# JanSpindler/NRC-HPM-Renderer

Hardware: AMD Instinct MI355X
Metric: Msamples/s + ms/frame at 1080p, 256^3 cloud (NRC path) (higher is better)
Workload: dtype f16 (fp16 MFMA operands, fp32 accumulate; fp32 integrator)

## Files before the change

### nrc-hpm-renderer_amd/csrc/nrc_api.hip

```cpp
#include <algorithm>
#include <array>
#include <atomic>
#include <chrono>
#include <cmath>
#include <cstdio>
#include <cstdlib>
#include <cstring>
#include <fstream>
#include <map>
#include <memory>
#include <mutex>
#include <random>
#include <string>
#include <thread>
#include <unordered_map>
#include <vector>

#include <dlfcn.h>
#include <rccl/rccl.h>

#include "nrc_integrator.hpp"
#include "nrc_mlp.hpp"
#include "nrc_checkpoint.hpp"
#include "nrc_occupancy.hpp"
#include "nrc_schedule.hpp"
#include "nrc_volume_keys.hpp"
#include "build_id.h"

namespace nrc {

static thread_local std::string g_last_error;

namespace {
constexpr size_t kGuardBytes = 4096;
struct AllocInfo {
    void* base;
    size_t bytes;
    std::string what;
};
struct AllocRegistry {
    std::mutex mu;
    std::unordered_map<void*, AllocInfo> live;
    bool poison = debug_value("poison_alloc", 0) != 0;
    bool guard = debug_value("guard_alloc", 0) != 0;
    unsigned long long violations = 0;
    std::string first_violation;
};
std::atomic<int> g_live_allocations{0};
AllocRegistry& alloc_registry()
{
    static AllocRegistry r;
    return r;
}
size_t guard_damage(const AllocInfo& a, std::string* where)
{
    std::vector<unsigned char> g(2 * kGuardBytes);
    if (hipMemcpy(g.data(), a.base, kGuardBytes, hipMemcpyDeviceToHost) != hipSuccess) return 0;
    if (hipMemcpy(g.data() + kGuardBytes, (char*)a.base + kGuardBytes + a.bytes, kGuardBytes, hipMemcpyDeviceToHost) != hipSuccess) return 0;
    size_t bad = 0;
    long first = -1;
    for (size_t i = 0; i < g.size(); i++)
        if (g[i] != 0xA5) { bad++; if (first < 0) first = (long)i; }
    if (bad && where)
        *where = a.what + " (" + std::to_string(a.bytes) + " B): " + std::to_string(bad) + " canary bytes overwritten, first at offset " +
                 (first < (long)kGuardBytes ? std::to_string(first - (long)kGuardBytes) : "+" + std::to_string(a.bytes + (size_t)first - kGuardBytes)) ;
    return bad;
}
}

void dev_alloc(void** p, size_t bytes, const char* what)
{
    AllocRegistry& r = alloc_registry();
    if (!r.guard) {
        NRC_HIP(hipMalloc(p, bytes));
        g_live_allocations++;
        if (r.poison && bytes) NRC_HIP(hipMemset(*p, 0xFF, bytes));
        return;
    }
    const size_t padded = (bytes + 255) & ~(size_t)255;
    void* base = nullptr;
    NRC_HIP(hipMalloc(&base, padded + 2 * kGuardBytes));
    NRC_HIP(hipMemset(base, 0xA5, padded + 2 * kGuardBytes));
    *p = (char*)base + kGuardBytes;
    g_live_allocations++;
    if (bytes) NRC_HIP(hipMemset(*p, r.poison ? 0xFF : 0x00, bytes));
    std::lock_guard<std::mutex> lock(r.mu);
    r.live[*p] = AllocInfo{base, bytes, what ? what : ""};
}

void dev_free(void* p)
{
    if (!p) return;
    g_live_allocations--;
    AllocRegistry& r = alloc_registry();
    if (!r.guard) {
        (void)hipFree(p);
        return;
    }
    AllocInfo a{nullptr, 0, ""};
    {
        std::lock_guard<std::mutex> lock(r.mu);
        auto it = r.live.find(p);
        if (it == r.live.end()) { (void)hipFree(p); return; }
        a = it->second;
        r.live.erase(it);
    }
    (void)hipDeviceSynchronize();
    AllocInfo chk = a;
// ... 1099 lines not shown
    unsigned long long* for_launch() const { return on ? d_count.get() : nullptr; }
    void set(bool enable, hipStream_t s) { on = enable; NRC_HIP(hipMemsetAsync(d_count, 0, 8, s)); }
    unsigned long long read(hipStream_t s) const
    {
        unsigned long long v = 0;
        NRC_HIP(hipMemcpyAsync(&v, d_count, 8, hipMemcpyDeviceToHost, s));
        NRC_HIP(hipStreamSynchronize(s));
        return v;
    }
};

struct PinnedRandom {
    float r[4] = {0, 0, 0, 0};
    bool have = false;
    void set(const float* r4) { std::memcpy(r, r4, 16); have = true; }
    bool take(float* frame_random) { if (have) std::memcpy(frame_random, r, 16); return std::exchange(have, false); }
};

static bool path_keys(const SceneDev& scene, uint32_t n_cameras, const nrc_camera* cameras, const float* times, uint32_t frames_per_camera,
                      std::vector<KeyTime>* keys)
{
    if (n_cameras == 0) return false;
    if (cameras == nullptr) fail("render_path: cameras is NULL");
    if (frames_per_camera == 0) fail("render_path: frames_per_camera must be at least 1");
    for (uint32_t i = 0; times != nullptr && i < n_cameras; i++) keys->push_back(scene.key_time(times[i], "render_path_timed"));
    return true;
}

static void export_framebuffer(const char* path, const float* d_rgba, uint32_t w, uint32_t h, hipStream_t s)
{
    std::vector<float> host((size_t)w * h * 4);
    NRC_HIP(hipMemcpyAsync(host.data(), d_rgba, host.size() * 4, hipMemcpyDeviceToHost, s));
    NRC_HIP(hipStreamSynchronize(s));
    write_exr(path, host, w, h);
}

class Renderer {
public:
    Renderer(uint32_t w, uint32_t h, bool blend, const nrc_camera& cam, const nrc_config& cfg, const nrc_scene& scene,
             Cache& cache, const nrc_tile* tile, hipStream_t s)
        : w_(w), h_(h), cam_(to_dev(cam)), cfg_(cfg), cache_(cache), stream_(s), blend_(blend), rng_(cfg.seed)
    {
        if (w == 0 || h == 0) fail("render size must be non-zero");
        if (((size_t)w * h) % 16 != 0) fail("NRC requires inferCount to be a multiple of 16");
        frame_ = make_frame(w, h, tile);
        tile_ = tile ? *tile : nrc_tile{0, 1, w, h, 1};
        prepare_hot_tiles(frame_, &hot_finder_);
        nq_ = query_count(w, h);
        scene_.upload(scene);
        calc_train_subset(cfg.train_batch_count * cache.train_batch_size());
        tg_.spp = cfg.train_spp;
        tg_.ray_length = (cfg.compat_fix & NRC_FIX_Q2_TRAIN_RAY_LEN) ? cfg.train_ray_length : 1u;
        tg_.ring_size = (uint32_t)(cfg.train_ring_buf_size * (float)(tg_.tw * tg_.th));
        const size_t px = (size_t)w * h, T = (size_t)tg_.tw * tg_.th;
        for (GenSet& g : gen_) {
            g.primary = alloc<float>(px * 4, "primary image"); g.info = alloc<float>(px, "info image");
            g.origin = alloc<float>(px * 4, "vertex origin image"); g.dir = alloc<float>(px * 4, "vertex direction image");
            g.infer_in = alloc<float>((size_t)nq_ * 5, "inference queries"); g.infer_out = alloc<float>((size_t)nq_ * 3, "inference radiance");
            if (!debug_switch("no_live_list")) g.live = alloc<uint32_t>((size_t)nq_ + 1, "live-query list");
            g.prep_done.create(); g.comp_done.create();
        }
        d_out_ = alloc<float>(px * 4, "framebuffer");
        if (cfg.self_train > 1u) fail("self_train must be 0 or 1");
        self_train_ = cfg.self_train != 0u;
        const size_t TS = T * tg_.spp;
        for (TrainSet& t : train_) {
            t.train_in = alloc<float>(T * 5, "training inputs"); t.train_target = alloc<float>(T * 3, "training targets");
            if (self_train_) {
                t.tail_q = alloc<float>(TS * 5, "tail queries"); t.tail_rec = alloc<float>(TS * 4, "tail records");
                t.tail_y = alloc<float>(TS * 3, "tail radiance");
            }
            t.infer_done.create(); t.train_done.create();
        }
        if (self_train_) cache.mlp().reserve_side_slot((uint32_t)TS);
        ring_entries_ = std::max<size_t>(T, tg_.ring_size);
        d_ring_ = alloc<uint32_t>(2 + ring_entries_ * 6, "train ring");
        d_scratch_ = alloc<uint32_t>(2 * T + 4, "train-ray scratch");
        fetch_.d_count = alloc<unsigned long long>(1, "fetch counter");
        mask_.d_tile_mask = alloc<uint32_t>(tile_mask_words(w, h), "tile mask");
        static_assert(kFlightStates % 32 == 0, "one bit per state, in whole words");
        mask_.d_flight_bits = alloc<uint32_t>((size_t)kFlightStates / 32 + 2, "flight bits");
        mask_.d_flight_sel = alloc<uint32_t>(1 + kFlightListMax, "flight selection");
        zero_dead_queries_ = debug_switch("zero_dead_queries");
        n_slots_ = camera_slots(w, h);
        if (n_slots_ > kOrderSlotMask) fail("render size: more 8x8 tiles than the launch order can address");
        d_tile_cost_ = alloc<uint32_t>(n_slots_, "tile costs");
        for (auto& o : d_tile_order_) o = alloc<uint32_t>(n_slots_, "tile order");
        {
            std::vector<uint32_t> ident(n_slots_);
            for (uint32_t i = 0; i < n_slots_; i++) ident[i] = i;
            for (auto& o : d_tile_order_) NRC_HIP(hipMemcpy(o, ident.data(), ident.size() * 4, hipMemcpyHostToDevice));
        }
        ev_order_done_ = make_event(hipEventDisableTiming);
        {
            hipDeviceProp_t prop{};
            int dev = 0;
            NRC_HIP(hipGetDevice(&dev));
            NRC_HIP(hipGetDeviceProperties(&prop, dev));
            std::string arch = prop.gcnArchName;
            arch = arch.substr(0, arch.find(':'));
            sched_ = ScheduleTuner(device_xcds() == 8, nrc::schedule_key(arch, prop.multiProcessorCount, device_xcds(), cfg,
                                                                    (unsigned long long)scene.nx * scene.ny * scene.nz, w, h, tile_.global_w,
                                                                    tile_.global_h, cache.train_batch_size(), tg_.ray_length));
        }
        mask_.cam = cam;
        if (!debug_switch("single_stream")) {
            int lo = 0, hi = 0;
            NRC_HIP(hipDeviceGetStreamPriorityRange(&lo, &hi));
            stream_b_ = make_stream(hi);
            stream_c_ = make_stream(hi);
            stream_d_ = make_stream(hi);
            if (train_paths_are_long(tg_)) {
                for (TraceSet& q : trace_) {
                    q.stream = make_stream(hi);
                    q.ev_trace_done = make_event(hipEventDisableTiming);
                    q.ev_staged = make_event(hipEventDisableTiming);
                    q.train_start = alloc<float>(T * 6, "staged start vertices");
                    q.in_stage = alloc<float>(T * 5, "staged training inputs");
                    q.target_stage = alloc<float>(T * 3, "staged training targets");
                    if (self_train_) {
                        q.tail_q_stage = alloc<float>(TS * 5, "staged tail queries");
                        q.tail_rec_stage = alloc<float>(TS * 4, "staged tail records");
                    }
                }
            }
        }
        std::vector<uint32_t> ring(2 + ring_entries_ * 6, 0);
        for (size_t r = 0; r < ring_entries_; r++) { float one = 1.0f; std::memcpy(&ring[2 + 6 * r + 5], &one, 4); }
        NRC_HIP(hipMemcpy(d_ring_, ring.data(), ring.size() * 4, hipMemcpyHostToDevice));
        cache_.init(nq_, gen_[0].infer_in, gen_[0].infer_out, train_[0].train_in, train_[0].train_target, s);
    }

    ~Renderer()
    {
        (void)hipDeviceSynchronize();
        cache_.forget(this);
    }

    void render(bool train, bool may_defer = false, bool mask_tiles = false)
    {
        if (train) cache_.poll_comm();
        if (ev_idx_.must_grow(ev_pool_.size())) {
            std::array<Event, 10> set;
            for (auto& e : set) e = make_event(hipEventDefault);
            ev_pool_.push_back(std::move(set));
        }
        sched_.step(TunerStep{frame_index_, ev_idx_.used, ev_pool_.size(), ev_idx_.last, ev_idx_.epoch, stage_events_, stream_c_ != nullptr}, *this);
        frame_.camera_priority_low = sched_.now().pri != 0 ? 1u : 0u;
        const Event* ev_ = ev_pool_[ev_idx_.take()].data();
        const float blend_factor = 1.0f / (float)blend_index_;
        const bool pinned = pinned_random_.take(frame_.random);
        if (!pinned && have_next_random_) { std::memcpy(frame_.random, next_random_, 16); have_next_random_ = false; }
        else if (!pinned) draw_random(frame_.random);
        if (blend_) blend_index_++;
        hipStream_t A = stream_, B = stream_b_ ? stream_b_ : stream_, Cs = stream_c_ ? stream_c_ : stream_;
        hipStream_t D = stream_d_ ? stream_d_ : B;
        mask_.update(scene_, &frame_, A, mask_tiles);
        const int pp = (int)(frame_index_ & 1u);
        const int gp = (int)(frame_index_ % (uint64_t)kGenSets);
        GenSet& g = gen_[gp];
        TrainSet& t = train_[pp];
        last_gen_ = gp; last_train_ = pp;
        if (frame_index_ >= (uint64_t)kGenSets) {
            if (Cs != A) NRC_HIP(hipStreamWaitEvent(A, g.comp_done.ev, 0));
            if (D != A && Cs == A) NRC_HIP(hipStreamWaitEvent(A, g.prep_done.ev, 0));
        }
        const int tq = (int)(frame_index_ % (uint64_t)kTraceSets);
        TraceSet& q = trace_[tq];
        const bool long_trace = q.stream != nullptr;
        if (long_trace) { if (frame_index_ >= (uint64_t)kTraceSets) NRC_HIP(hipStreamWaitEvent(D, q.ev_staged, 0)); }
        else if (frame_index_ >= 2 && D != B) NRC_HIP(hipStreamWaitEvent(D, t.train_done.ev, 0));
        if (cost_order_ && order_pending_ && frame_index_ >= order_pending_frame_ + (uint64_t)sched_.now().lag) {
            if (D != A) NRC_HIP(hipStreamWaitEvent(A, ev_order_done_, 0));
            order_cur_ ^= 1;
            order_pending_ = false;
        }
        const bool sample_cost = cost_order_ && !order_pending_ && (frame_index_ % kOrderEvery == 0 || order_resample_);
        if (sample_cost) order_resample_ = false;
        frame_.tile_order = cost_order_ ? d_tile_order_[order_cur_].get() : nullptr;
        frame_.tile_cost = sample_cost ? d_tile_cost_.get() : nullptr;
        frame_.tile_cost_keep = order_fresh_ > 0 ? 0u : kOrderKeep;
        if (sample_cost && order_fresh_ > 0) order_fresh_--;
        frame_.hot_front = frame_.hot_n = 0u;
        const bool promote = hot_promote_ && frame_.tile_mask != nullptr && frame_.flight_mode == 1u && frame_.flight_n > 0;
        if (promote) {
            last_hot_predicted_ = next_known_ && std::memcmp(known_random_, frame_.random, 16) == 0;
            last_hot_list_ = promote_hot_tiles(&frame_, &hot_finder_);
            const float* nr = next_random_;
            if (have_hint_) nr = hint_random_;
            else if (!have_next_random_) { draw_random(next_random_); have_next_random_ = true; }
            std::memcpy(known_random_, nr, 16);
        }
        have_hint_ = false;
        next_known_ = promote;
        last_hot_ = promote;
        frame_.live_list = frame_.live_count = nullptr;
        if (g.live != nullptr && cache_.wants_live_list()) {
            frame_.live_count = g.live;
            frame_.live_list = frame_.live_count + 1;
        }
        frame_.skip_dead_queries = (!zero_dead_queries_ && frame_.live_list != nullptr && (cache_.encodes_in_kernel() || cache_.model_has_grid())) ? 1u : 0u;
        {
            LaunchTailScope tail(A, ev_[1], ev_[0]);
            launch_gen_rays(scene_.d, cam_, frame_, cfg_.primary_ray_length, cfg_.primary_ray_prob, g.primary, g.info, g.origin, g.dir,
                            g.infer_in, fetch_.for_launch(), tg_, full_vertex_images_, A);
            tail.finish();
        }
        if (D != A) NRC_HIP(hipStreamWaitEvent(D, ev_[1], 0));
        if (Cs != A) NRC_HIP(hipStreamWaitEvent(Cs, ev_[1], 0));
        const hipEvent_t prep_done = g.prep_done.select(stage_events_, ev_[2]);
        const bool pre_encode = train && D != B && frame_index_ >= 2 && !long_trace && cache_.can_pre_encode(this);
        const bool self_train = train && self_train_ && tg_.ring_size > 0;
        float* tail_q = self_train ? (long_trace ? q.tail_q_stage : t.tail_q).get() : nullptr;
        float* tail_rec = self_train ? (long_trace ? q.tail_rec_stage : t.tail_rec).get() : nullptr;
        {
            LaunchTailScope tail(D);
            if (!pre_encode) tail.arm(prep_done);
            launch_prep_train(scene_.d, frame_, tg_, g.info, g.origin, g.dir, d_ring_, d_scratch_, long_trace ? q.in_stage : t.train_in,
                              t.train_target, D, long_trace ? q.train_start.get() : nullptr, long_trace ? nullptr : tail_q,
                              long_trace ? nullptr : tail_rec);
            if (pre_encode) {
                cache_.pre_encode(t.train_in, pp, D);
                tail.arm(prep_done);
            }
            tail.finish();
        }
        if (long_trace) {
            hipStream_t T = q.stream;
            NRC_HIP(hipStreamWaitEvent(T, prep_done, 0));
            {
                LaunchTailScope tail(T, q.ev_trace_done);
                launch_train_trace(scene_.d, frame_, tg_, q.train_start, q.target_stage, T, tail_q, tail_rec);
                tail.finish();
            }
            NRC_HIP(hipStreamWaitEvent(B, q.ev_trace_done, 0));
            const size_t nT = (size_t)tg_.tw * tg_.th;
            NRC_HIP(hipMemcpyAsync(t.train_in, q.in_stage, nT * 5 * sizeof(float), hipMemcpyDeviceToDevice, B));
            if (!self_train) {
                NRC_HIP(hipMemcpyAsync(t.train_target, q.target_stage, nT * 3 * sizeof(float), hipMemcpyDeviceToDevice, B));
                NRC_HIP(hipEventRecord(q.ev_staged, B));
            }
        } else if (B != D) NRC_HIP(hipStreamWaitEvent(B, prep_done, 0));
        if (sample_cost) {
            LaunchTailScope tail(D, ev_order_done_);
            launch_tile_order(d_tile_cost_, n_slots_, d_tile_order_[order_cur_ ^ 1], w_, D,
                              sched_.xcd_ok() ? (uint32_t)sched_.now().window : 0u, hot_promote_ ? kHotTilesMax / 4u : 0u);
            tail.finish();
            order_pending_ = true;
            order_pending_frame_ = frame_index_;
        }
        if (pending_comp_.valid) launch_pending_composite(D);
        if (B != Cs && frame_index_ > 0) NRC_HIP(hipStreamWaitEvent(Cs, train_[pp ^ 1].train_done.ev, 0));
        cache_.acquire(this, Cs, B);
        cache_.bind(nq_, g.infer_in, g.infer_out, t.train_in, t.train_target);
        const hipEvent_t infer_done = t.infer_done.select(stage_events_, ev_[3]);
        cache_.infer_all(nullptr, Cs, true, frame_.live_list, frame_.live_count, infer_done);
        const hipEvent_t train_done = t.train_done.select(stage_events_, ev_[5]);
        if (self_train) {
            const uint32_t nT = tg_.tw * tg_.th;
            cache_.mlp().infer(tail_q, t.tail_y, nT * tg_.spp, true, B, false, nullptr, nullptr, Mlp::kSideSlot);
            launch_self_train_combine(nT, tg_.spp, tail_rec, t.tail_y, t.train_target, B);
            if (long_trace) NRC_HIP(hipEventRecord(q.ev_staged, B));
            last_tail_train_ = pp; last_tail_trace_ = long_trace ? tq : -1;
        }
        if (train) cache_.train_all(B, (B != Cs && frame_index_ > 0) ? train_[pp ^ 1].infer_done.ev : nullptr,
                                    B != Cs ? infer_done : nullptr, train_done);
        else NRC_HIP(hipEventRecord(train_done, B));
        const bool defer = may_defer && sched_.now().defer != 0 && D != Cs && D != A;
        if (defer) {
            pending_comp_.valid = true;
            pending_comp_.gp = gp;
            pending_comp_.blend = blend_factor;
            pending_comp_.show_nrc = show_nrc_;
            pending_comp_.ev_infer = infer_done;
            pending_comp_.ev_stage = stage_events_ ? ev_[4] : g.comp_done.own;
            pending_comp_.frame = frame_;
        } else {
            if (consumer_pending_) {
                NRC_HIP(hipStreamWaitEvent(Cs, ev_consumer_, 0));
                consumer_pending_ = false;
            }
            if (last_comp_event_ && last_comp_stream_ != Cs) NRC_HIP(hipStreamWaitEvent(Cs, last_comp_event_, 0));
            if (D != Cs) NRC_HIP(hipStreamWaitEvent(Cs, prep_done, 0));
            const hipEvent_t comp_done = g.comp_done.select(stage_events_, ev_[4]);
// ... 350 lines not shown
            if (!self_train_) fail("buffers 9-11 belong to a self-training renderer (nrc_config.self_train)");
            const TrainSet& tt = train_[last_tail_train_];
            const TraceSet* st = last_tail_trace_ >= 0 ? &trace_[last_tail_trace_] : nullptr;
            p = which == 9 ? (st ? st->tail_q_stage : tt.tail_q) : which == 10 ? (st ? st->tail_rec_stage : tt.tail_rec) : tt.tail_y;
            b = T * tg_.spp * (which == 9 ? 20 : (which == 10 ? 16 : 12));
            break;
        }
        default: fail("bad buffer id");
        }
        if (bytes) *bytes = b;
        return p;
    }
    float* public_queries(const float* tiled, uint32_t floats_per_query, const float* info)
    {
        DevBuf<float>& dst = floats_per_query == 5 ? d_pub_in_ : d_pub_out_;
        if (!dst) dst = alloc<float>((size_t)w_ * h_ * floats_per_query, "public query copy");
        launch_query_layout(frame_, floats_per_query, tiled, dst, stream_, info);
        NRC_HIP(hipStreamSynchronize(stream_));
        return dst;
    }
    const float* framebuffer()
    {
        wait_frame(stream_);
        return d_out_;
    }
    void wait_frame(hipStream_t consumer)
    {
        if (frame_index_ > 0)
            NRC_HIP(hipStreamWaitEvent(consumer, gen_[(frame_index_ - 1) % (uint64_t)kGenSets].comp_done.ev, 0));
    }
    void release_frame(hipStream_t consumer)
    {
        if (!ev_consumer_) ev_consumer_ = make_event(hipEventDisableTiming);
        NRC_HIP(hipEventRecord(ev_consumer_, consumer));
        consumer_pending_ = true;
    }
    bool is_blending() const { return blend_; }
    void set_full_vertex_images(bool on) { full_vertex_images_ = on; }
    size_t vertex_image_bytes() const { return (full_vertex_images_ ? (size_t)w_ * h_ : (size_t)tg_.tw * tg_.th) * 32; }
    const float* framebuffer_unordered() const { return d_out_; }
    const TrainGrid& train_grid() const { return tg_; }
    hipStream_t stream() const { return stream_; }

private:
    template <class T>
    static DevBuf<T> alloc(size_t count, const char* what)
    {
        DevBuf<T> b;
        b.alloc(count * sizeof(T), what);
        NRC_HIP(hipMemset(b, 0, count * sizeof(T)));
        return b;
    }

    void calc_train_subset(uint32_t train_pixel_count)
    {
        const uint32_t sq = (uint32_t)std::sqrt((double)train_pixel_count);
        for (uint32_t factor = sq; factor >= 2; factor--) {
            if (train_pixel_count % factor == 0) {
                const uint32_t other = train_pixel_count / factor;
                const uint32_t bigger = std::max(factor, other), smaller = std::min(factor, other);
                if (w_ > h_) { tg_.tw = bigger; tg_.th = smaller; }
                else { tg_.tw = smaller; tg_.th = bigger; }
                tg_.x_dist = w_ / tg_.tw;
                const uint32_t y_dist = h_ / tg_.th;
                tg_.y_dist = (cfg_.compat_fix & NRC_FIX_Q1_TRAIN_Y_DIST) ? y_dist : tg_.x_dist;
                return;
            }
        }
        fail("Could not find suitable division of trainPixelCount");
    }

    uint32_t w_, h_;
    DevCamera cam_;
    DevFrame frame_{};
    nrc_config cfg_;
    Cache& cache_;
    hipStream_t stream_;
    Stream stream_b_, stream_c_, stream_d_;
    SceneDev scene_;
    TrainGrid tg_{};
    nrc_tile tile_{};
    uint32_t nq_ = 0;
    uint64_t frame_index_ = 0;
    bool self_train_ = false, full_vertex_images_ = false, zero_dead_queries_ = false;
    struct StageEnd {
        Event own;
        hipEvent_t ev = nullptr;
        void create() { own = make_event(hipEventDisableTiming); ev = own; }
        hipEvent_t select(bool timed, hipEvent_t frame_event) { return ev = timed ? frame_event : own.get(); }
    };
#ifndef NRC_GEN_SETS
#define NRC_GEN_SETS 6
#endif
    static constexpr int kGenSets = NRC_GEN_SETS;
    struct GenSet {
        DevBuf<float> primary, info, origin, dir;
        DevBuf<float> infer_in, infer_out;
        DevBuf<uint32_t> live;
        StageEnd prep_done, comp_done;
    };
    struct TrainSet {
        DevBuf<float> train_in, train_target;
        DevBuf<float> tail_q, tail_rec, tail_y;
        StageEnd infer_done, train_done;
    };
    static constexpr int kTraceSets = 4;
    struct TraceSet {
        Stream stream;
        Event ev_trace_done;
        Event ev_staged;
        DevBuf<float> train_start;
        DevBuf<float> in_stage, target_stage;
        DevBuf<float> tail_q_stage, tail_rec_stage;
    };
    GenSet gen_[kGenSets];
    TrainSet train_[2];
    TraceSet trace_[kTraceSets];
    int last_gen_ = 0, last_train_ = 0, last_tail_train_ = 0, last_tail_trace_ = -1;
    DevBuf<uint32_t> d_ring_, d_scratch_;
    size_t ring_entries_ = 0;
    DevBuf<float> d_pub_in_, d_pub_out_;
    DevBuf<float> d_gather_;
    size_t gather_bytes_ = 0;
    FetchCounter fetch_;
    DevBuf<float> d_out_;
    bool blend_;
    uint32_t blend_index_ = 1;
    uint32_t show_nrc_ = 1;
    struct PendingComposite {
        bool valid = false;
        int gp = 0;
        float blend = 1.0f;
        uint32_t show_nrc = 0;
        hipEvent_t ev_infer = nullptr, ev_stage = nullptr;
        DevFrame frame;
    };
    PendingComposite pending_comp_;
    hipEvent_t last_comp_event_ = nullptr;
    hipStream_t last_comp_stream_ = nullptr;
    Event ev_consumer_;
    bool consumer_pending_ = false;
    Event ev_clear_;
    Event ev_path_;
    std::mt19937 rng_;
    PinnedRandom pinned_random_;
    float next_random_[4] = {0, 0, 0, 0}, hint_random_[4] = {0, 0, 0, 0};
    bool have_next_random_ = false, have_hint_ = false;
    void draw_random(float* r4)
    {
        std::uniform_real_distribution<float> u(0.0f, 1.0f);
        for (int k = 0; k < 4; k++) r4[k] = u(rng_);
    }
    DevBuf<uint32_t> d_tile_cost_;
    DevBuf<uint32_t> d_tile_order_[2];
    uint32_t n_slots_ = 0;
    Event ev_order_done_;
    bool cost_order_ = true, order_pending_ = false;
    int order_cur_ = 0;
    uint64_t order_pending_frame_ = 0;
    static constexpr uint64_t kOrderEvery = 4;
    static constexpr uint32_t kOrderKeep = 4;
    bool order_resample_ = false;
    int order_fresh_ = 2;
    EmptySpaceMask mask_;
    HotTileFinder hot_finder_;
    HotList last_hot_list_;
    bool hot_promote_ = true, next_known_ = false, last_hot_ = false, last_hot_predicted_ = false;
    float known_random_[4] = {0, 0, 0, 0};
    Event ev_slot_[2][1 + kTraceSets];
    bool slot_left_[2] = {false, false};
    std::vector<std::array<Event, 10>> ev_pool_;
    EventPoolIndex ev_idx_;
    bool stage_events_ = true;
    ScheduleTuner sched_;
};

class McRenderer {
public:
    McRenderer(uint32_t w, uint32_t h, uint32_t path_length, bool blend, const nrc_camera& cam, const nrc_scene& scene,
               const nrc_tile* tile, hipStream_t s)
        : w_(w), h_(h), path_length_(path_length), blend_(blend), cam_(to_dev(cam)), stream_(s), rng_(1337)
    {
        if (w == 0 || h == 0) fail("render size must be non-zero");
        frame_ = make_frame(w, h, tile);
        prepare_hot_tiles(frame_, &hot_finder_);
        scene_.upload(scene);
        const size_t px = (size_t)w * h;
        d_out_.alloc(px * 4 * sizeof(float), "d_out_"); NRC_HIP(hipMemset(d_out_, 0, px * 16));
        d_info_.alloc(px * sizeof(float), "d_info_"); NRC_HIP(hipMemset(d_info_, 0, px * 4));
        fetch_.d_count.alloc(sizeof(unsigned long long), "d_fetch_"); NRC_HIP(hipMemset(fetch_.d_count, 0, 8));
        mask_.d_tile_mask.alloc((size_t)tile_mask_words(w, h) * sizeof(uint32_t), "d_tile_mask_");
        mask_.d_flight_bits.alloc(((size_t)kFlightStates / 32 + 2) * sizeof(uint32_t), "d_flight_bits_");
        mask_.d_flight_sel.alloc((1 + kFlightListMax) * sizeof(uint32_t), "d_flight_sel_");
        for (auto& e : ev_) e = make_event(hipEventDefault);
        mask_.cam = cam;
        xcd_window_ = device_xcds() == 8 ? 2u : 0u;
        n_slots_ = camera_slots(w, h);
        d_tile_cost_.alloc((size_t)n_slots_ * sizeof(uint32_t), "d_tile_cost_");
        d_tile_order_.alloc((size_t)n_slots_ * sizeof(uint32_t), "d_tile_order_");
        std::vector<uint32_t> ident(n_slots_);
        for (uint32_t i = 0; i < n_slots_; i++) ident[i] = i;
        NRC_HIP(hipMemcpy(d_tile_order_, ident.data(), (size_t)n_slots_ * 4, hipMemcpyHostToDevice));
    }
    void set_empty_skip(bool on) { mask_.empty_skip = on; mask_.dirty = true; }
    void render(bool mask_tiles = false)
    {
        mask_.update(scene_, &frame_, stream_, mask_tiles);
        const float blend_factor = 1.0f / (float)blend_index_;
        if (!pinned_random_.take(frame_.random)) { std::uniform_real_distribution<float> u(0.0f, 1.0f); for (float& r : frame_.random) r = u(rng_); }
        if (blend_) blend_index_++;
        const bool sample_cost = cost_order_ && (frame_index_ % 4 == 0 || order_fresh_ == 2);
        frame_.tile_order = cost_order_ ? d_tile_order_.get() : nullptr;
        frame_.tile_cost = sample_cost ? d_tile_cost_.get() : nullptr;
        frame_.tile_cost_keep = order_fresh_ > 0 ? 0u : 4u;
        if (sample_cost && order_fresh_ > 0) order_fresh_--;
        frame_.hot_front = frame_.hot_n = 0u;
        if (hot_promote_ && frame_.tile_mask != nullptr && frame_.flight_mode == 1u && frame_.flight_n > 0) promote_hot_tiles(&frame_, &hot_finder_);
        NRC_HIP(hipEventRecord(ev_[0], stream_));
        launch_mc_render(scene_.d, cam_, frame_, path_length_, blend_factor, d_out_, d_info_, fetch_.for_launch(), stream_);
        NRC_HIP(hipEventRecord(ev_[1], stream_));
        if (sample_cost) launch_tile_order(d_tile_cost_, n_slots_, d_tile_order_, w_, stream_,
                                           xcd_window_, hot_promote_ ? kHotTilesMax / 4u : 0u);
        frame_index_++;
        timed_ = true;
    }
    void set_cost_order(bool on) { cost_order_ = on; }
    void set_camera(const nrc_camera& c)
    {
        cam_ = to_dev(c);
        mask_.cam = c;
        mask_.dirty = true;
        order_fresh_ = 2;
        blend_index_ = 1;
        NRC_HIP(hipMemsetAsync(d_out_, 0, (size_t)w_ * h_ * 16, stream_));
    }
    void set_scene_params(const nrc_scene& s) { scene_.set_params(s); mask_.dirty = true; }
    void set_volume(const void* src, uint32_t nx, uint32_t ny, uint32_t nz, int format, bool on_device)
    {
        scene_.check_volume(src, nx, ny, nz, format);
        swap_volume([&] { scene_.write_slot(0, src, format, on_device, stream_); });
    }
    void set_volume_bricks(const int32_t* origins, const void* bricks, uint32_t n, int format, bool on_device)
    {
        scene_.check_bricks(origins, bricks, n, format, on_device);
        swap_volume([&] { scene_.write_slot_bricks(0, origins, bricks, n, format, on_device, stream_); });
    }
    void set_volume_keys(const void* src, uint32_t n, uint32_t nx, uint32_t ny, uint32_t nz, int format, bool on_device)
    {
        scene_.check_keys(src, n, nx, ny, nz, format);
        NRC_HIP(hipStreamSynchronize(stream_));
        scene_.set_keys(src, n, format, on_device, stream_);
// ... 784 lines not shown
```

### nrc-hpm-renderer_amd/csrc/nrc_integrator.hip

```cpp
#include "nrc_integrator.hpp"

#include <cstdlib>
#include <string>

#include "nrc_math.h"
#include "nrc_volume_keys.hpp"

#ifndef NRC_CAMERA_WAVES_PER_SIMD
#define NRC_CAMERA_WAVES_PER_SIMD 5
#endif

namespace nrc {
namespace {

struct V3 {
    float x, y, z;
};
__device__ __forceinline__ V3 v3(float x, float y, float z) { return V3{x, y, z}; }
__device__ __forceinline__ V3 add(V3 a, V3 b) { return v3(a.x + b.x, a.y + b.y, a.z + b.z); }
__device__ __forceinline__ V3 sub(V3 a, V3 b) { return v3(a.x - b.x, a.y - b.y, a.z - b.z); }
__device__ __forceinline__ V3 mul(V3 a, float s) { return v3(a.x * s, a.y * s, a.z * s); }
__device__ __forceinline__ V3 neg(V3 a) { return v3(-a.x, -a.y, -a.z); }
__device__ __forceinline__ float dot(V3 a, V3 b) { return nrc_fmaf_(a.z, b.z, nrc_fmaf_(a.y, b.y, a.x * b.x)); }
__device__ __forceinline__ float length(V3 a) { return sqrtf(dot(a, a)); }
// ... 788 lines not shown
                y = (t >> 16) * 8u + (lane >> 3);
                inside = lx < fr.w && y < fr.h;
                hot_wave = true;
            } else {
                inside = pixel_of_launch_slot(fr, d - kHotTilesMax, &lx, &y, &slot);
                const uint32_t t = __builtin_amdgcn_readfirstlane(((y >> 3) << 16) | (lx >> 3));
                bool is_hot = false;
#pragma unroll
                for (uint32_t k = 0; k < kHotTilesMax; k++) is_hot |= (k < hot_n) & (t == hot[k]);
                if (is_hot) return false;
            }
        } else {
            inside = pixel_of_launch_slot(fr, d, &lx, &y, &slot);
        }
    }
    *lx_ = lx; *y_ = y; *slot_ = slot; *inside_ = inside; *hot_wave_ = hot_wave;
    return true;
}

__device__ __forceinline__ void store_tile_cost(const DevFrame& fr, uint32_t slot, unsigned long long cycles)
{
    uint32_t c = (uint32_t)min(cycles, 0xffffffffull);
    if (fr.tile_cost_keep != 0u) {
        const uint32_t old = fr.tile_cost[slot];
        c = max(c, old - (old >> fr.tile_cost_keep));
    }
    fr.tile_cost[slot] = c;
}

__device__ __forceinline__ void count_fetches(unsigned long long* counter, uint32_t n)
{
    if (counter == nullptr) return;
    unsigned long long v = n;
#pragma unroll
    for (int off = 32; off >= 1; off >>= 1) v += __shfl_xor(v, off);
    if ((threadIdx.x & 63u) == 0) atomicAdd(counter, v);
}

typedef float out_f4 __attribute__((ext_vector_type(4)));
__device__ __forceinline__ void out_store(float4* p, float4 v)
{
    *p = v;
}
__device__ __forceinline__ void out_store(float* p, float v)
{
    *p = v;
}

#ifndef NRC_GEN_WAVES_PER_SIMD
#define NRC_GEN_WAVES_PER_SIMD NRC_CAMERA_WAVES_PER_SIMD
#endif
template <bool COUNT>
__global__ __launch_bounds__(64 * CAMERA_WAVES_PER_BLOCK, NRC_GEN_WAVES_PER_SIMD) void k_gen_rays(DevScene sc, DevCamera cam, DevFrame fr, uint32_t primary_ray_length,
                                                 float primary_ray_prob, float4* __restrict__ primary,
                                                 float* __restrict__ info, float4* __restrict__ origin,
                                                 float4* __restrict__ dirs, float* __restrict__ infer_in,
                                                 unsigned long long* fetch_counter, TrainGrid tg, int full_vertex_images)
{
    camera_wave_priority(fr);
    const unsigned long long t_start = __builtin_amdgcn_s_memtime();
    __shared__ uint32_t s_occ[kOccMaxWords];
    uint32_t lx = 0, y = 0, slot = 0;
    bool inside, hot_wave;
    if (!camera_wave_tile(fr, &lx, &y, &slot, &inside, &hot_wave)) return;
#ifdef NRC_LOOP_PROFILE
    const uint32_t wave_id = blockIdx.x * CAMERA_WAVES_PER_BLOCK + (threadIdx.x >> 6);
    if ((threadIdx.x & 63u) == 0 && wave_id < 65536u) {
        unsigned xcc, hw;
        asm volatile("s_getreg_b32 %0, hwreg(HW_REG_XCC_ID)" : "=s"(xcc));
        asm volatile("s_getreg_b32 %0, hwreg(HW_REG_HW_ID)" : "=s"(hw));
        g_wave_times[4 * wave_id] = wall_clock64();
        g_wave_times[4 * wave_id + 2] = xcc;
        g_wave_times[4 * wave_id + 3] = hw;
    }
#endif
    if (__ballot(inside) == 0ull) return;
    CtxT<COUNT> c{sc, 0.0f, 0u};
    const uint32_t gx = global_x(fr, lx);
    const float u = (float)gx * fr.inv_gw, v = (float)y * fr.inv_gh;
    const float seed_uv = random2(u, v);
    if (tile_mask_clear(fr, lx, y)) {
        c.rng = random2(seed_uv, random4(fr.random));
        if (!tile_has_capped_state(fr, inside, c.rng)) {
            if (inside) {
                V3 ro, rd;
                camera_ray(cam, u, v, &ro, &rd);
                const V3 e = sample_env_dir(sc, rd);
                const size_t pix = (size_t)y * fr.w + lx;
                out_store(&primary[pix], make_float4(e.x, e.y, e.z, 1.0f));
                out_store(&info[pix], 0.0f);
                if (fr.skip_dead_queries == 0u) {
                    float* qo = infer_in + query_index(fr.w, lx, y) * 5u;
#pragma unroll
                    for (int k = 0; k < 5; k++) out_store(&qo[k], 0.0f);
                }
            }
            if (fr.tile_cost != nullptr && !hot_wave && (threadIdx.x & 63u) == 0) store_tile_cost(fr, slot, __builtin_amdgcn_s_memtime() - t_start);
#ifdef NRC_LOOP_PROFILE
            if (inside && full_vertex_images != 0) reinterpret_cast<float*>(origin)[4 * ((size_t)y * fr.w + lx) + 3] = 0.0f;
            if ((threadIdx.x & 63u) == 0 && wave_id < 65536u) g_wave_times[4 * wave_id + 1] = wall_clock64();
#endif
            return;
        }
    }
    c.occ = load_occupancy_per_wave(sc, s_occ);
    V3 ro, rd;
    camera_ray(cam, u, v, &ro, &rd);
    c.rng = random2(seed_uv, random4(fr.random));
    const bool enter = inside;
    V3 entry = ro, ex;
    {
#ifdef NRC_LOOP_PROFILE
        c.fee_kind = 0;
#endif
        find_entry_exit(c, sel(enter, ro, v3(0.0f, 0.0f, 0.0f)), sel(enter, rd, v3(0.0f, 0.0f, 1.0f)), &entry, &ex);
#ifdef NRC_LOOP_PROFILE
        c.fee_kind = 1;
#endif
    }
    const bool entered = enter && !(sky_sdf(sc, entry) > 100000.0f);
    if (inside) {
        const V3 e = sample_env_dir(sc, rd);
        out_store(&primary[(size_t)y * fr.w + lx], make_float4(e.x, e.y, e.z, 1.0f));
    }
    V3 light = v3(0, 0, 0);
    V3 cur = entry, dir = rd;
    float factor = 1.0f;
    bool did_scatter = false, walking = entered;
    for (int i = 0;; i++) {
        if (__ballot(walking) == 0ull) break;
        bool vexit = false;
        const V3 nc = delta_track<true>(c, cur, dir, &vexit, walking);
        cur = sel(walking, nc, cur);
        walking &= !vexit;
        did_scatter |= walking;
        factor = walking ? factor * 0.5f : factor;
        if (__ballot(walking) == 0ull) break;
        const V3 ts = trace_scene<true>(c, cur, dir, walking);
        if (walking) {
            light = add(light, mul(ts, factor));
            dir = new_ray_dir(c, dir, true);
            if ((uint32_t)i >= primary_ray_length) {
                if (c.rand(1.0f) >= primary_ray_prob || i == 128) walking = false;
            }
        }
    }
    if (inside) {
        const size_t pix = (size_t)y * fr.w + lx;
        float q[5] = {0.0f, 0.0f, 0.0f, 0.0f, 0.0f};
        if (entered) {
            bool on_grid = full_vertex_images != 0;
            if (!on_grid) {
                const uint32_t qx = tg.x_dist ? lx / tg.x_dist : 0u, qy = tg.y_dist ? y / tg.y_dist : 0u;
                on_grid = (qx * tg.x_dist == lx) & (qy * tg.y_dist == y) & (qx < tg.tw) & (qy < tg.th);
            }
            if (on_grid) {
                origin[pix] = make_float4(cur.x, cur.y, cur.z, 0.0f);
                dirs[pix] = make_float4(dir.x, dir.y, dir.z, 0.0f);
            }
            if (did_scatter) {
                nrc_query(sc, cur, dir, q);
                out_store(&primary[pix], make_float4(light.x, light.y, light.z, factor));
            }
        }
        out_store(&info[pix], did_scatter ? 1.0f : 0.0f);
        if (fr.skip_dead_queries == 0u || (entered && did_scatter)) {
            float* qo = infer_in + query_index(fr.w, lx, y) * 5u;
// ... 1277 lines not shown
```

### nrc-hpm-renderer_amd/csrc/nrc_integrator.hpp

```cpp
#pragma once
#include "nrc_common.hpp"
#include "nrc_hot_tiles.hpp"

namespace nrc {

struct DevScene {
    const uint8_t* density;
    uint32_t nx, ny, nz;
    float fnx, fny, fnz;
    float size[3], half_size[3], inv_size[3];
    float len2size;
    float density_factor, inv_max_density, g;
    float dir_light_dir[3], dir_light_strength;
    float point_light_pos[3], point_light_strength, point_light_color[3];
    const float* env;
    uint32_t env_w, env_h;
    float env_strength;
    const uint32_t* occ_bits;
    uint32_t occ_shift, occ_gx, occ_gy, occ_words;
};
constexpr uint32_t kOccMaxWords = 2048;

struct DevCamera {
    float m[16];
    float pos[3];
};

struct DevFrame {
    float random[4];
    uint32_t w, h;
    uint32_t x_offset, x_stride;
    uint32_t x_block_log2;
    float inv_gw, inv_gh;
    const uint32_t* tile_mask;
    uint32_t flight_mode, flight_n;
    uint32_t flight_list[8];
    const uint32_t* flight_bits;
    const uint32_t* tile_order;
    uint32_t* tile_cost;
    uint32_t tile_cost_keep;
    uint32_t hot_front, hot_n;
    uint32_t hot[8];
    uint32_t* live_list;
    uint32_t* live_count;
    uint32_t raise_priority;
    uint32_t camera_priority_low;
    uint32_t skip_dead_queries;
};
constexpr uint32_t kOrderSlotMask = 0x00ffffffu;

struct DevProjView {
    float m[16];
};

struct TrainGrid {
    uint32_t tw, th, x_dist, y_dist, spp, ray_length, ring_size;
};

void launch_gen_rays(const DevScene& sc, const DevCamera& cam, const DevFrame& fr, uint32_t primary_ray_length,
                     float primary_ray_prob, float* primary, float* info, float* origin, float* dir, float* infer_in,
                     unsigned long long* fetch_counter, const TrainGrid& tg, bool full_vertex_images, hipStream_t s);

void launch_query_layout(const DevFrame& fr, uint32_t floats_per_query, const float* tiled, float* linear, hipStream_t s,
                         const float* info = nullptr);
uint32_t query_count(uint32_t w, uint32_t h);
struct BoxList {
    const float* boxes;
    uint32_t n_host;
    const uint32_t* n_dev;
    uint32_t grid;
};
void launch_tile_mask(const BoxList& b, const DevProjView& pv, const DevFrame& fr, uint32_t* mask, hipStream_t s);
uint32_t tile_mask_words(uint32_t w, uint32_t h);
void launch_tile_mask_tiles(const BoxList& b, const DevProjView& pv, const DevFrame& fr, void* rects, uint32_t* mask, hipStream_t s);

struct VolumeRebuild {
    uint8_t* density;
    uint32_t* occ_bits;
    float* boxes;
    uint32_t* n_boxes;
    uint32_t nx, ny, nz;
    uint32_t occ_shift, occ_gx, occ_gy, occ_gz, occ_words;
    double lo[3], vs[3];
};
uint32_t volume_box_capacity(uint32_t nx, uint32_t ny, uint32_t nz);
size_t volume_scratch_bytes(uint32_t nx, uint32_t ny, uint32_t nz);
void launch_volume_rebuild(const void* src, int format, const VolumeRebuild& v, void* scratch, hipStream_t s);
size_t volume_brick_index_bytes(uint32_t nx, uint32_t ny, uint32_t nz);
void launch_volume_rebuild_bricks(const int32_t* origins, const void* bricks, uint32_t n_bricks, int format, const VolumeRebuild& v, void* scratch,
                                  uint32_t* brick_index, hipStream_t s);
void launch_volume_quantize(const float* src, uint8_t* dst, size_t n, hipStream_t s);
void launch_volume_rebuild_lerp(const uint8_t* key_a, const uint8_t* key_b, uint32_t W, const VolumeRebuild& v, void* scratch, hipStream_t s);
constexpr uint32_t kFlightStates = 1u << 23;
void launch_flight_table(float* table, hipStream_t s);
void launch_flight_select(const float* table, float lambda, uint32_t* count_and_list, uint32_t* bits, hipStream_t s);
uint32_t camera_slots(uint32_t w, uint32_t h);
void launch_tile_order(const uint32_t* cost, uint32_t n_slots, uint32_t* order, uint32_t w, hipStream_t s, uint32_t xcd_window = 0, uint32_t workgroups_in_front = 0);

void launch_mc_render(const DevScene& sc, const DevCamera& cam, const DevFrame& fr, uint32_t path_length,
                      float blend_factor, float* out_rgba, float* info, unsigned long long* fetch_counter, hipStream_t s);

void launch_prep_train(const DevScene& sc, const DevFrame& fr, const TrainGrid& tg, const float* info,
                       const float* origin, const float* dir, uint32_t* ring, uint32_t* scratch, float* train_in,
                       float* train_target, hipStream_t s, float* start = nullptr, float* tail_query = nullptr, float* tail_rec = nullptr);
void launch_train_trace(const DevScene& sc, const DevFrame& fr, const TrainGrid& tg, const float* start, float* train_target, hipStream_t s,
                        float* tail_query = nullptr, float* tail_rec = nullptr);
void launch_self_train_combine(uint32_t T, uint32_t spp, const float* tail_rec, const float* tail_y, float* train_target, hipStream_t s);
bool train_paths_are_long(const TrainGrid& tg);

void integrator_set_wave_priority_raise(int on);
void launch_composite(const DevFrame& fr, uint32_t show_nrc, float blend_factor, const float* primary,
                      const float* info, const float* infer_out, float* out_rgba, hipStream_t s, uint32_t* live_count_reset = nullptr);

void launch_compare(const float* ref_rgba, const float* own_rgba, uint32_t n_pixels, double* d_scratch, float* d_result5,
                    hipStream_t s);

void launch_compare_sharded_1(const float* ref_rgba, const float* own_rgba, uint32_t n_pixels, double* d_scratch, hipStream_t s);
void launch_compare_sharded_2(const float* ref_rgba, const float* own_rgba, uint32_t n_pixels, double* d_scratch, hipStream_t s);
void launch_compare_sharded_3(double* d_scratch, float* d_result5, hipStream_t s);
void launch_pad_columns(const float* local, uint32_t lw, uint32_t h, uint32_t max_lw, float* padded, hipStream_t s);
void launch_assemble_columns(const float* gathered, uint32_t world, uint32_t block_log2, uint32_t gw, uint32_t h, uint32_t max_lw, float* out,
                             hipStream_t s);
void launch_test_math(int fn, const float* a, const float* b, uint32_t n, float* out, float* out2, hipStream_t s);
void launch_test_rng(float u, float v, const float* frame_random4, uint32_t n, float* out, hipStream_t s);

}
```

Before: 9126.

## Skip rewriting sky pixels in masked tiles when the generation buffer still holds them

Adds per-generation-set bookkeeping (epoch plus the last hot-tile list) so that, when the tile mask is in force and nothing has invalidated the buffer, the ray-generation kernel leaves sky pixels of clear tiles in place instead of recomputing the camera ray and environment lookup. Tiles that were hot in the previous use of that buffer are marked stale and still get rewritten. This removes redundant environment sampling and stores for masked tiles. The risk is stale output if an invalidation path is missed; setting rewrite_sky forces the old behaviour.

```diff
diff --git a/nrc-hpm-renderer_amd/csrc/nrc_api.hip b/nrc-hpm-renderer_amd/csrc/nrc_api.hip
--- a/nrc-hpm-renderer_amd/csrc/nrc_api.hip
+++ b/nrc-hpm-renderer_amd/csrc/nrc_api.hip
@@ -24,6 +24,7 @@
 #include "nrc_checkpoint.hpp"
 #include "nrc_occupancy.hpp"
 #include "nrc_schedule.hpp"
+#include "nrc_sky_in_place.hpp"
 #include "nrc_volume_keys.hpp"
 #include "build_id.h"
 
@@ -1289,6 +1290,7 @@
         mask_.d_flight_bits = alloc<uint32_t>((size_t)kFlightStates / 32 + 2, "flight bits");
         mask_.d_flight_sel = alloc<uint32_t>(1 + kFlightListMax, "flight selection");
         zero_dead_queries_ = debug_switch("zero_dead_queries");
+        rewrite_sky_ = debug_switch("rewrite_sky");
         n_slots_ = camera_slots(w, h);
         if (n_slots_ > kOrderSlotMask) fail("render size: more 8x8 tiles than the launch order can address");
         d_tile_cost_ = alloc<uint32_t>(n_slots_, "tile costs");
@@ -1362,6 +1364,7 @@
         if (blend_) blend_index_++;
         hipStream_t A = stream_, B = stream_b_ ? stream_b_ : stream_, Cs = stream_c_ ? stream_c_ : stream_;
         hipStream_t D = stream_d_ ? stream_d_ : B;
+        if (mask_.dirty) sky_epoch_++;
         mask_.update(scene_, &frame_, A, mask_tiles);
         const int pp = (int)(frame_index_ & 1u);
         const int gp = (int)(frame_index_ % (uint64_t)kGenSets);
@@ -1407,6 +1410,19 @@
             frame_.live_list = frame_.live_count + 1;
         }
         frame_.skip_dead_queries = (!zero_dead_queries_ && frame_.live_list != nullptr && (cache_.encodes_in_kernel() || cache_.model_has_grid())) ? 1u : 0u;
+        if (frame_.skip_dead_queries != sky_skip_dead_) { sky_skip_dead_ = frame_.skip_dead_queries; sky_epoch_++; }
+        {
+            SkyFrame sf;
+            sf.epoch = sky_epoch_;
+            sf.mask_in_force = frame_.tile_mask != nullptr && frame_.flight_mode != 0u;
+            sf.list_known = promote;
+            sf.force_rewrite = rewrite_sky_;
+            if (promote) sf.hot = last_hot_list_;
+            const SkyDecision sd = sky_decide(&g.sky, sf);
+            frame_.sky_in_place = sd.in_place ? 1u : 0u;
+            frame_.sky_stale_n = sd.stale_n;
+            for (uint32_t k = 0; k < kHotTilesMax; k++) frame_.sky_stale[k] = sd.stale[k];
+        }
         {
             LaunchTailScope tail(A, ev_[1], ev_[0]);
             launch_gen_rays(scene_.d, cam_, frame_, cfg_.primary_ray_length, cfg_.primary_ray_prob, g.primary, g.info, g.origin, g.dir,
@@ -1923,7 +1939,7 @@
     nrc_tile tile_{};
     uint32_t nq_ = 0;
     uint64_t frame_index_ = 0;
-    bool self_train_ = false, full_vertex_images_ = false, zero_dead_queries_ = false;
+    bool self_train_ = false, full_vertex_images_ = false, zero_dead_queries_ = false, rewrite_sky_ = false;
     struct StageEnd {
         Event own;
         hipEvent_t ev = nullptr;
@@ -1939,6 +1955,7 @@
         DevBuf<float> infer_in, infer_out;
         DevBuf<uint32_t> live;
         StageEnd prep_done, comp_done;
+        SkyRecord sky;
     };
     struct TrainSet {
         DevBuf<float> train_in, train_target;
@@ -2008,6 +2025,8 @@
     HotList last_hot_list_;
     bool hot_promote_ = true, next_known_ = false, last_hot_ = false, last_hot_predicted_ = false;
     float known_random_[4] = {0, 0, 0, 0};
+    uint64_t sky_epoch_ = 1;
+    uint32_t sky_skip_dead_ = 0;
     Event ev_slot_[2][1 + kTraceSets];
     bool slot_left_[2] = {false, false};
     std::vector<std::array<Event, 10>> ev_pool_;
diff --git a/nrc-hpm-renderer_amd/csrc/nrc_integrator.hip b/nrc-hpm-renderer_amd/csrc/nrc_integrator.hip
--- a/nrc-hpm-renderer_amd/csrc/nrc_integrator.hip
+++ b/nrc-hpm-renderer_amd/csrc/nrc_integrator.hip
@@ -894,7 +894,15 @@
     if (tile_mask_clear(fr, lx, y)) {
         c.rng = random2(seed_uv, random4(fr.random));
         if (!tile_has_capped_state(fr, inside, c.rng)) {
-            if (inside) {
+            bool in_place = false;
+            if (fr.sky_in_place != 0u) {
+                const uint32_t t = __builtin_amdgcn_readfirstlane(((y >> 3) << 16) | (lx >> 3));
+                bool stale = false;
+#pragma unroll
+                for (uint32_t k = 0; k < kHotTilesMax; k++) stale |= (k < fr.sky_stale_n) & (t == fr.sky_stale[k]);
+                in_place = !stale;
+            }
+            if (inside && !in_place) {
                 V3 ro, rd;
                 camera_ray(cam, u, v, &ro, &rd);
                 const V3 e = sample_env_dir(sc, rd);
diff --git a/nrc-hpm-renderer_amd/csrc/nrc_integrator.hpp b/nrc-hpm-renderer_amd/csrc/nrc_integrator.hpp
--- a/nrc-hpm-renderer_amd/csrc/nrc_integrator.hpp
+++ b/nrc-hpm-renderer_amd/csrc/nrc_integrator.hpp
@@ -46,6 +46,8 @@
     uint32_t raise_priority;
     uint32_t camera_priority_low;
     uint32_t skip_dead_queries;
+    uint32_t sky_in_place, sky_stale_n;
+    uint32_t sky_stale[8];
 };
 constexpr uint32_t kOrderSlotMask = 0x00ffffffu;
 
diff --git a/nrc-hpm-renderer_amd/csrc/nrc_sky_in_place.hpp b/nrc-hpm-renderer_amd/csrc/nrc_sky_in_place.hpp
--- /dev/null
+++ b/nrc-hpm-renderer_amd/csrc/nrc_sky_in_place.hpp
@@ -0,0 +1,42 @@
+#pragma once
+#include <cstdint>
+
+#include "nrc_hot_tiles.hpp"
+
+namespace nrc {
+
+struct SkyRecord {
+    uint64_t epoch = 0;
+    bool complete = false;
+    HotList hot;
+};
+
+struct SkyFrame {
+    uint64_t epoch = 0;
+    bool mask_in_force = false;
+    bool list_known = false;
+    bool force_rewrite = false;
+    HotList hot;
+};
+
+struct SkyDecision {
+    bool in_place = false;
+    uint32_t stale_n = 0;
+    uint32_t stale[kHotTilesMax] = {};
+};
+
+inline SkyDecision sky_decide(SkyRecord* set, const SkyFrame& f)
+{
+    SkyDecision d;
+    if (!f.force_rewrite && f.mask_in_force && set->epoch == f.epoch && set->complete) {
+        d.in_place = true;
+        d.stale_n = set->hot.count;
+        for (uint32_t k = 0; k < d.stale_n; k++) d.stale[k] = set->hot.entries[k];
+    }
+    set->epoch = f.epoch;
+    set->complete = f.mask_in_force && f.list_known && f.hot.count <= kHotTilesMax;
+    set->hot = f.hot;
+    return d;
+}
+
+}
```

Result: no change. 9168, median of 6 (+0.5%).
